# Alabuta/RaytracingInOneWeekend

Hardware: AMD Instinct MI355X
Metric: Mrays/sec + frame wall-clock, huge-scene 1280x720x128spp @1/2/4/8 GPU (higher is better)
Workload: dtype f32; 1 GPU; huge-scene 1280x720x128spp (BASELINE config 3); scene=huge (486 spheres), width=1280, height=720, spp=128, max_depth=64, camera=reference, kernel=exact (bit-exact), cull, parallelism=row-interleaved x1, RCCL gather of f32 tiles, output=f32, hw_queues=8, hw_queues_env=4, deep_split=8, deep_min_items=33554432

## Files before the change

### raytracinginoneweekend_amd/csrc/rt_kernel.hip

```cpp
#include <hip/hip_runtime.h>
#include <float.h>
#include <stdint.h>

#include "rt_device.h"

namespace rt {

#define RT_TMIN 0.008f
#define RT_TMAX FLT_MAX

struct f3 { float x, y, z; };
__device__ __forceinline__ f3 mk(float x, float y, float z) { return {x, y, z}; }
__device__ __forceinline__ f3 operator+(f3 a, f3 b) { return {a.x + b.x, a.y + b.y, a.z + b.z}; }
__device__ __forceinline__ f3 operator-(f3 a, f3 b) { return {a.x - b.x, a.y - b.y, a.z - b.z}; }
__device__ __forceinline__ f3 operator*(f3 a, f3 b) { return {a.x * b.x, a.y * b.y, a.z * b.z}; }
__device__ __forceinline__ f3 operator*(f3 a, float s) { return {a.x * s, a.y * s, a.z * s}; }
__device__ __forceinline__ f3 operator/(f3 a, float s) { return {a.x / s, a.y / s, a.z / s}; }
__device__ __forceinline__ f3 adds(f3 a, float s) { return {a.x + s, a.y + s, a.z + s}; }
__device__ __forceinline__ float dot(f3 a, f3 b) { return a.x * b.x + a.y * b.y + a.z * b.z; }
__device__ __forceinline__ float length(f3 a) { return sqrtf(a.x * a.x + a.y * a.y + a.z * a.z); }
__device__ __forceinline__ f3 normalize(f3 a)
{
    float l = length(a);
    return fabsf(l) > FLT_MIN ? a / l : a;
// ... 1269 lines not shown
                        }
                    }
                }
            }
            stamp(3);
        }
        if constexpr (COUNT) {
            uint32_t r = trap_rem;
            for (int off = 32; off >= 1; off >>= 1) r += (uint32_t)__shfl_xor((int)r, off);
            wt.add_seg(r);
        }
        if (done) {
            RT_EV(EV_STORE);
            finish(col);
        }
    }

    if (COUNT && p.segments) {
        if (lane == 0) {
            atomicAdd(p.segments + 0, (unsigned long long)wt.seg);
            atomicAdd(p.segments + 1, (unsigned long long)wt.sph);
            atomicAdd(p.segments + 2, (unsigned long long)wt.box);
        }
    }
    if (STATS && p.dbg) {
        const uint32_t c[8] = {dbg_iters, dbg_refills, dbg.wave_blocks, dbg.lane_blocks, dbg.wave_roots,
                               dbg.lane_roots, lane == 0 ? (uint32_t)wt.seg : 0u, dbg.wave_member_blocks};
#pragma unroll
        for (int i = 0; i < 8; ++i) {
            unsigned long long v = c[i];
            for (int off = 32; off >= 1; off >>= 1) v += __shfl_xor(v, off);
            if (lane == 0) atomicAdd(p.dbg + i, v);
        }
#pragma unroll
        for (int i = 0; i < (int)EV_COUNT; ++i) {
            unsigned long long v = dbg.ev[i];
            for (int off = 32; off >= 1; off >>= 1) v += __shfl_xor(v, off);
            if (lane == 0) atomicAdd(p.dbg + kDbgEvBase + i, v);
        }
        if (lane == 0) {
            for (int i = 0; i < 5; ++i) atomicAdd(p.dbg + 8 + i, (unsigned long long)cyc[i]);
            atomicMax(p.dbg + 14, ~t_wave0);
            atomicAdd(p.dbg + 13, (unsigned long long)dbg_dealt);
        }
        const uint32_t w = blockIdx.x * (blockDim.x >> 6) + (threadIdx.x >> 6);
        if (lane == 0 && w < kDbgWaves) {
            const unsigned long long cy = cyc[0] + cyc[1] + cyc[2] + cyc[3] + cyc[4];
            p.dbg[16 + 4 * w] = DEEP ? ((unsigned long long)dbg_walks_nohint << 32 | dbg_walks)
                                     : (t_dry ? t_dry : __builtin_amdgcn_s_memrealtime());
            p.dbg[17 + 4 * w] = __builtin_amdgcn_s_memrealtime();
            p.dbg[18 + 4 * w] = (min(cy, 0xffffffffull) << 32) | (min(dbg_refills, 65535u) << 16) | min(dbg_iters, 65535u);
            p.dbg[19 + 4 * w] = ((unsigned long long)(__smid() & 0xffffu) << 48) |
                                ((unsigned long long)min(DEEP ? dbg_walks : dbg_iters_dry, 65535u) << 32) | (uint32_t)t_wave0;
        }
    }
}

template <int V, int CULL, bool STATS, bool COUNT, bool PAIRS = false>
__global__ __launch_bounds__(256, (kMinWaves<V, CULL, STATS>)) void render_kernel(const KParams p)
{
    render_body<V, CULL, STATS, COUNT, false, 4, PAIRS>(p);
}
template <int V, bool STATS, bool COUNT, int WPB>
__global__ __launch_bounds__(64 * WPB, (WPB == 8 && !STATS ? RT_DEEP_WIDE_WAVES : kMinWaves<V, 7, STATS>)) void render_deep_kernel(const KParams p)
{
    render_body<V, 7, STATS, COUNT, true, WPB, false>(p);
}

__device__ __forceinline__ float xs_gen(uint32_t &st)
{
    st ^= st << 13;
    st ^= st >> 17;
    st ^= st << 5;
    return (float)st * (1.f / 4294967296.f);
}
__device__ __forceinline__ f3 xs_unit_sphere(uint32_t &st)
{
    f3 v;
    do {
        const float x = xs_gen(st) * 2.f - 1.f;
        const float y = xs_gen(st) * 2.f - 1.f;
        const float z = xs_gen(st) * 2.f - 1.f;
        v = mk(x, y, z);
    } while (v.x * v.x + v.y * v.y + v.z * v.z > 0x1.000002p+0f && st != 0u);
    return v;
}

__global__ __launch_bounds__(256) void compat_kernel(const KCompat p)
{
    const uint32_t lane = threadIdx.x & 63u;
    const float4 *shade = p.shade;
    const uint8_t *kinds = reinterpret_cast<const uint8_t *>(shade + 2 * p.n_spheres);
    const f3 org = mk(p.org[0], p.org[1], p.org[2]), llc = mk(p.llc[0], p.llc[1], p.llc[2]);
    const f3 hor = mk(p.hor[0], p.hor[1], p.hor[2]), ver = mk(p.ver[0], p.ver[1], p.ver[2]);
    const float fW = (float)p.W, fH = (float)p.H;

    uint32_t cnext = 0, cend = 0;
    bool exhausted = false, alive = false, fresh = false;
    uint32_t i = 0, x = 0, y = 0, s = 0, depth = 0, rng = 0;
    f3 o = mk(0.f, 0.f, 0.f), d = o, att = o, col = o;
    uint32_t segs = 0, tests = 0;
    for (;;) {
        uint64_t need = ballot(!alive);
        while (need && !exhausted) {
            if (cnext >= cend) {
                uint32_t c = 0;
                if (lane == 0) c = atomicAdd(p.ctr, 1u);
                c = __builtin_amdgcn_readfirstlane(c);
                if (c >= p.n_chunks) { exhausted = true; break; }
                cnext = c * 64u;
                cend = min(cnext + 64u, p.n_pixels);
            }
            const uint32_t avail = cend - cnext;
            const uint32_t rank = __builtin_amdgcn_mbcnt_hi((uint32_t)(need >> 32),
                                                            __builtin_amdgcn_mbcnt_lo((uint32_t)need, 0u));
            if (!alive && rank < avail) {
                i = cnext + rank;
                const uint32_t rr = i / p.W;
                x = i - rr * p.W;
                y = p.row_offset + rr * p.row_stride;
                rng = x + y * p.W + p.seed;
                s = 0;
                col = mk(0.f, 0.f, 0.f);
                alive = fresh = true;
            }
            cnext += min((uint32_t)__popcll(need), avail);
            need = ballot(!alive);
        }
        if (ballot(alive) == 0) break;
        if (!alive) continue;
        if (fresh) {
            const float u = ((float)x + xs_gen(rng)) / fW;
            const float v = ((float)y + xs_gen(rng)) / fH;
            o = org;
            d = (llc + hor * u) + ver * (1.f - v);
            att = mk(1.f, 1.f, 1.f);
            depth = 0;
            fresh = false;
        }
        bool done = false;
        f3 c = mk(0.f, 0.f, 0.f);
        if (depth >= p.max_depth) {
            done = true;
        } else {
            ++segs;
            const float a = d.x * d.x + d.y * d.y + d.z * d.z;
            float tmax = RT_TMAX;
            uint32_t ib = 0xffffffffu;
            for (uint32_t k = 0; k < p.n_spheres; ++k) {
                const float4 sf = shade[2 * k];
                const float ocx = o.x - sf.x, ocy = o.y - sf.y, ocz = o.z - sf.z;
                const float b = ocx * d.x + ocy * d.y + ocz * d.z;
                const float cc = ocx * ocx + ocy * ocy + ocz * ocz - sf.w * sf.w;
                const float disc = b * b - a * cc;
                if (disc > 0.f) {
                    const float q = sqrtf(disc);
                    float t = (-b - q) / a;
                    if (!(t < tmax && t > RT_TMIN)) t = (-b + q) / a;
                    if (t < tmax && t > RT_TMIN) { tmax = t; ib = k; }
                }
            }
            tests += p.n_spheres;
            ++depth;
            if (ib == 0xffffffffu) {
                const float tt = normalize(d).y * .5f + .5f;
                c = (mk(1.f, 1.f, 1.f) * (1.f - tt) + mk(.5f, .7f, 1.f) * tt) * att;
                done = true;
            } else {
                const float4 sf = shade[2 * ib], md = shade[2 * ib + 1];
                const uint32_t kind = kinds[ib];
                const f3 hp = o + d * tmax;
                const f3 hn = (hp - mk(sf.x, sf.y, sf.z)) / sf.w;
                bool valid = true;
                f3 nd;
                if (kind == 0u) {
                    nd = hn + normalize(xs_unit_sphere(rng));
                } else if (kind == 1u) {
                    const f3 refl = reflect(normalize(d), hn);
                    nd = refl + normalize(xs_unit_sphere(rng)) * md.w;
                    valid = dot(nd, hn) > 0.f;
                } else {
                    const f3 ud = normalize(d);
                    f3 outward = mk(-hn.x, -hn.y, -hn.z);
                    float ri = md.w;
                    float cosv = dot(ud, hn);
                    if (cosv <= 0.f) {
                        outward = outward * -1.f;
                        ri = 1.f / ri;
                        cosv *= -1.f;
                    }
                    const f3 refr = refract(ud, outward, ri);
                    float prob = 1.f;
                    if (refr.x * refr.x + refr.y * refr.y + refr.z * refr.z > 0.f) prob = schlick(ri, cosv);
                    nd = xs_gen(rng) < prob ? reflect(ud, hn) : refr;
                }
                if (!valid) {
                    done = true;
                } else {
                    o = hp;
                    d = nd;
                    att = att * mk(md.x, md.y, md.z);
                    if (depth >= p.max_depth) done = true;
                }
            }
        }
        if (done) {
            col = col + c;
            if (++s == p.spp) {
                col = col / (float)p.spp;
                const uint32_t row = p.full_frame ? y : i / p.W;
                float *dst = p.out + ((size_t)row * p.W + x) * 3u;
                dst[0] = col.x;
                dst[1] = col.y;
                dst[2] = col.z;
                alive = false;
            } else {
                fresh = true;
            }
        }
    }
    if (p.segments) {
        const unsigned long long cv[2] = {segs, tests};
        for (int k = 0; k < 2; ++k) {
            unsigned long long v = cv[k];
            for (int off = 32; off >= 1; off >>= 1) v += __shfl_xor(v, off);
            if (lane == 0) atomicAdd(p.segments + k, v);
        }
    }
}

__global__ __launch_bounds__(256) void accumulate_kernel(const KAccum k)
{
    const uint32_t i = blockIdx.x * blockDim.x + threadIdx.x;
    if (i == 0 && k.seg_to)
        for (int c = 0; c < 3; ++c) {
            k.seg_to[c] += k.seg_from[c];
            k.seg_from[c] = 0ull;
        }
    if (k.queue_reset)
        for (uint32_t w = i; w < k.queue_words; w += gridDim.x * blockDim.x) {
            if (k.deep_over && (w & (kQueueStride - 1u)) == kDeepCount && k.queue_reset[w] > k.deep_rcap)
                *k.deep_over = k.deep_key;
            k.queue_reset[w] = 0u;
        }
    if (i >= k.n_pixels) return;
    const bool sky = i >= k.sky_pos0;
    if (sky) {
        if (!k.last || k.part == 1) return;
    } else if (k.part) {
        const bool flagged = k.deep_px[i];
        if (k.part == 1 && flagged) return;
        if (k.part == 2 && !flagged) return;
        if (k.part != 1 && flagged) k.deep_px[i] = 0;
    }
    const uint32_t ni = k.block_perm ? (k.block_perm[i >> 6] << 6) | (i & 63u) : i;
    f3 acc;
    if (sky) acc = mk(k.slots[3 * i], k.slots[3 * i + 1], k.slots[3 * i + 2]);
    else if (k.first) acc = mk(0.f, 0.f, 0.f);
    else acc = mk(k.acc[3 * ni], k.acc[3 * ni + 1], k.acc[3 * ni + 2]);
    auto ld = [&](uint32_t s) {
        const float *v = k.slots + ((size_t)s * k.n_pixels + i) * 3u;
        return mk(v[0], v[1], v[2]);
    };
    if (sky) {
    } else if (k.paired) {
        for (uint32_t b = 0; b < k.n_blocks; ++b) acc = acc + (ld(2u * b) + ld(2u * b + 1u));
        for (uint32_t t = 4u * k.n_blocks; t < k.n_samples; ++t) acc = acc + ld(t - 2u * k.n_blocks);
    } else {
        uint32_t s = 0;
        for (; s < 4u * k.n_blocks; s += 4u) acc = acc + ((ld(s) + ld(s + 1u)) + (ld(s + 2u) + ld(s + 3u)));
        for (; s < k.n_samples; ++s) acc = acc + ld(s);
    }
    if (!k.last) {
        k.acc[3 * ni] = acc.x; k.acc[3 * ni + 1] = acc.y; k.acc[3 * ni + 2] = acc.z;
        return;
    }
    const f3 col = acc / (float)k.spp;
    uint32_t x, rr;
    {
        const uint32_t tiled_px = k.tiled_rows * k.W;
        if (ni < tiled_px) {
            uint32_t t = ni >> 6, w = ni & 63u;
            uint32_t ty = t / k.tiles_x, tx = t - ty * k.tiles_x;
            x = (tx << k.tile_lw) + (w & ((1u << k.tile_lw) - 1u));
            rr = (ty << (6u - k.tile_lw)) + (w >> k.tile_lw);
        } else {
            uint32_t jj = ni - tiled_px;
            rr = jj / k.W;
            x = jj - rr * k.W;
            rr += k.tiled_rows;
        }
    }
    const uint32_t row = k.full_frame ? k.row_offset + rr * k.row_stride : rr;
    const size_t o = ((size_t)row * k.W + x) * 3u;
    k.out[o] = col.x; k.out[o + 1] = col.y; k.out[o + 2] = col.z;
    if (k.out_u8) {
        const double g = (double)(1.f / 2.2f);
        k.out_u8[o] = (uint8_t)(255.f * (float)pow((double)col.x, g));
        k.out_u8[o + 1] = (uint8_t)(255.f * (float)pow((double)col.y, g));
        k.out_u8[o + 2] = (uint8_t)(255.f * (float)pow((double)col.z, g));
    }
}

#ifndef RT_SKY_CAP
#define RT_SKY_CAP 2
#endif
__global__ __launch_bounds__(256) void sky_kernel(const KSky p)
{
    const FrameConsts &fc = p.fc;
    const uint32_t t = blockIdx.x * 256u + threadIdx.x;
    const bool live = t < p.n_pix;
    uint32_t px, rr;
    pixel_of(fc, p.pos0 + (live ? t : 0u), px, rr, p.block_perm);
    const uint32_t py = fc.row_offset + rr * fc.row_stride;
    const uint64_t inc_data = ((uint64_t)fc.inc_data_hi << 32) | fc.inc_data_lo;
    const uint64_t inc_cam = ((uint64_t)fc.inc_cam_hi << 32) | fc.inc_cam_lo;
    const uint64_t key0 = (uint64_t)(py * fc.W + px) * fc.spp;
    const uint32_t spp = fc.spp, full_end = spp & ~3u;
    const float fW = fc.fW, fH = fc.fH, rW = fc.rW, rH = fc.rH;
    const bool dw = fc.div_fast & 1u, dh = fc.div_fast & 2u;
    const f3 org = mk(fc.org[0], fc.org[1], fc.org[2]), llc = mk(fc.llc[0], fc.llc[1], fc.llc[2]);
    const f3 hor = mk(fc.hor[0], fc.hor[1], fc.hor[2]), ver = mk(fc.ver[0], fc.ver[1], fc.ver[2]);
    f3 acc = mk(0.f, 0.f, 0.f), pa = acc, pb = acc;
    uint32_t s = live ? 0u : spp;
    bool started = false;
    uint64_t rc = 0;
    float uu = 0.f, vv = 0.f;
    Dbg dbg{};
    const uint64_t cd1 = inc_data * (kPcgMul + 1u), cd2 = cd1 * kPcgMul + inc_data, cc = inc_cam * (kPcgMul + 1u);
    const uint64_t mm = kPcgMul * kPcgMul;
    uint64_t km = key0 * kPcgMul, kmm = km * kPcgMul;
    const float ux = div_const((float)px, fW, rW, dw), vy = div_const((float)py, fH, rH, dh);
    while (ballot(s < spp)) {
        if (s < spp) {
            if (!started) {
                rc = km + cc;
                const float xu = fminf((float)pcg_out(km + cd1), 0x1.fffffep31f) * 0x1p-32f;
                const float xv = fminf((float)pcg_out(kmm + cd2), 0x1.fffffep31f) * 0x1p-32f;
                uu = ux + div_const(xu, fW, rW, dw);
                vv = vy + div_const(xv, fH, rH, dh);
                km += kPcgMul;
                kmm += mm;
                started = true;
            }
            bool got;
            const f3 r = random_in_unit_sphere_capped<false, RT_SKY_CAP>(rc, inc_cam, got, dbg);
            if (got) {
                const f3 rd = r * fc.lens;
                const f3 off = mk(uu * rd.x, vv * rd.y, 0.f);
                f3 d = ((llc + hor * uu) + ver * (1.f - vv)) - off;
                if (fc.corrected) d = d - org;
                const float a = d.x * d.x + d.y * d.y + d.z * d.z;
                float uy;
                if (!ballot(!(a >= 0x1p-40f && a <= 0x1p40f))) {
                    const float l = sqrt_scaled(a);
                    const float y0 = __builtin_amdgcn_rcpf(l);
                    uy = div_ray(d.y, RayDiv{l, fmaf(fmaf(-l, y0, 1.f), y0, y0), 1u});
                } else {
                    uy = normalize(d).y;
                }
                const float tt = .5f * uy + 1.f;
                const f3 col = mk(1.f, 1.f, 1.f) * (1.f - tt) + mk(.5f, .7f, 1.f) * tt;
                const bool tail = s >= full_end;
                const uint32_t j = s & 3u;
                const f3 sum = pa + col;
                const bool odd = !tail && (j & 1u);
                pa = mk(odd ? sum.x : col.x, odd ? sum.y : col.y, odd ? sum.z : col.z);
                const bool first_pair = !tail && j == 1u;
                pb = mk(first_pair ? pa.x : pb.x, first_pair ? pa.y : pb.y, first_pair ? pa.z : pb.z);
                const bool fold = tail || j == 3u;
                const f3 add = pb + pa;
                const f3 fa = acc + mk(tail ? col.x : add.x, tail ? col.y : add.y, tail ? col.z : add.z);
                acc = mk(fold ? fa.x : acc.x, fold ? fa.y : acc.y, fold ? fa.z : acc.z);
                ++s;
                started = false;
            }
        }
    }
    if (live) {
        float *o = p.sums + 3u * (size_t)t;
        o[0] = acc.x;
        o[1] = acc.y;
        o[2] = acc.z;
    }
    if (p.segments) {
        const uint32_t n = lanes(live);
        if ((threadIdx.x & 63u) == 0u && n) atomicAdd(p.segments, (unsigned long long)n * spp);
    }
}

__global__ __launch_bounds__(256) void epilogue_rgb8_kernel(const float *in, uint8_t *out, uint64_t n)
{
    const uint64_t i = (uint64_t)blockIdx.x * blockDim.x + threadIdx.x;
    if (i >= n) return;
    const double g = (double)(1.f / 2.2f);
    out[i] = (uint8_t)(255.f * (float)pow((double)in[i], g));
}

__global__ __launch_bounds__(256) void wave_gen_kernel(const KWave w)
{
    const KParams &p = w.p;
    const FrameConsts &fc = p.fc;
    const uint32_t gid = blockIdx.x * 256u + threadIdx.x;
    if (gid >= w.n_chunk) return;
    const uint32_t I = w.item_begin + gid;
    const uint32_t ls = udiv(I, fc.div_n_pixels);
    const uint32_t pix = I - ls * fc.n_pixels;
    uint32_t px, rr;
    pixel_of(fc, pix, px, rr, nullptr);
    const uint32_t py = fc.row_offset + rr * fc.row_stride;
    const uint32_t sm = fc.sample_begin + ls;
    const uint64_t inc_data = ((uint64_t)fc.inc_data_hi << 32) | fc.inc_data_lo;
    const uint64_t inc_cam = ((uint64_t)fc.inc_cam_hi << 32) | fc.inc_cam_lo;
    const uint64_t km = ((uint64_t)(py * fc.W + px) * fc.spp + sm) * kPcgMul;
    uint64_t rng = km + inc_data * (kPcgMul + 1u);
    uint64_t rc = km + inc_cam * (kPcgMul + 1u);
    const bool fw = fc.div_fast & 1u, fh = fc.div_fast & 2u;
    const float u = div_const((float)px, fc.fW, fc.rW, fw);
    const float v = div_const((float)py, fc.fH, fc.rH, fh);
    const float uu = u + div_const(canonical(rng, inc_data), fc.fW, fc.rW, fw);
    const float vv = v + div_const(canonical(rng, inc_data), fc.fH, fc.rH, fh);
    const f3 r = random_in_unit_sphere(rc, inc_cam);
    const f3 rd = r * fc.lens;
    const f3 off = mk(uu * rd.x, vv * rd.y, 0.f);
    const f3 org = mk(fc.org[0], fc.org[1], fc.org[2]);
    const f3 o = org + off;
    f3 d = ((mk(fc.llc[0], fc.llc[1], fc.llc[2]) + mk(fc.hor[0], fc.hor[1], fc.hor[2]) * uu) +
            mk(fc.ver[0], fc.ver[1], fc.ver[2]) * (1.f - vv)) - off;
    if (fc.corrected) d = d - org;
    const RayQueue &q = w.out;
    q.f[0 * w.cap + gid] = o.x; q.f[1 * w.cap + gid] = o.y; q.f[2 * w.cap + gid] = o.z;
    q.f[3 * w.cap + gid] = d.x; q.f[4 * w.cap + gid] = d.y; q.f[5 * w.cap + gid] = d.z;
    q.f[6 * w.cap + gid] = 1.f; q.f[7 * w.cap + gid] = 1.f; q.f[8 * w.cap + gid] = 1.f;
    q.rng[gid] = rng;
    q.item[gid] = I;
    q.depth[gid] = 0u;
    if (gid == 0) *q.count = w.n_chunk;
}

template <int CULL, bool COUNT>
__global__ __launch_bounds__(256, 6) void wave_bounce_kernel(const KWave w)
{
    const KParams &p = w.p;
    extern __shared__ float4 lds_blob[];
    for (uint32_t i = threadIdx.x; i < p.lds_units; i += blockDim.x) lds_blob[i] = p.blob[i];
    __syncthreads();
    const float4 *blob = lds_blob;
    const float4 *geo = blob;
    const uint32_t *sidx = reinterpret_cast<const uint32_t *>(blob + p.n_geo);
    const float4 *clus = blob + p.clus_offset;
    __shared__ TransposeLds s_tw[4];
    TransposeLds *tw = &s_tw[threadIdx.x >> 6];
    const uint64_t inc_data = ((uint64_t)p.fc.inc_data_hi << 32) | p.fc.inc_data_lo;
    const RayQueue &qi = w.in, &qo = w.out;
    const uint32_t n = *qi.count;
    const uint32_t cap = w.cap;
    WaveTally<COUNT> wt;
    Dbg dbg{};
    for (uint32_t base = blockIdx.x * 256u; base < n; base += gridDim.x * 256u) {
        const uint32_t j = base + threadIdx.x;
        const bool live = j < n;
        const uint32_t jj = live ? j : 0u;
        f3 o = mk(qi.f[0 * cap + jj], qi.f[1 * cap + jj], qi.f[2 * cap + jj]);
        f3 d = mk(qi.f[3 * cap + jj], qi.f[4 * cap + jj], qi.f[5 * cap + jj]);
        f3 att = mk(qi.f[6 * cap + jj], qi.f[7 * cap + jj], qi.f[8 * cap + jj]);
        uint64_t rng = qi.rng[jj];
        const uint32_t I = qi.item[jj];
        uint32_t depth = qi.depth[jj];
        const bool seg = live && depth < p.max_depth;
        const float a = d.x * d.x + d.y * d.y + d.z * d.z;
        const uint64_t segm = ballot(seg);
        const RayDiv rd = ray_div(a, segm, p.fast_roots);
        Hit h = closest_hit<false, CULL, false, COUNT>(p, geo, sidx, clus, o, d, rd, dbg, wt, seg, segm, CULL ? tw : nullptr,
                                                        no_hit());
        if (!seg) h = Hit{kNoHit};
        {
            const uint32_t ns = lanes(seg);
            wt.add_seg(ns);
            wt.add_sph((uint64_t)ns * p.n_always);
        }
        bool done = false, cont = false;
        f3 col = mk(0.f, 0.f, 0.f);
        if (live) {
            if (!seg) {
                done = true;
            } else {
                const float t = h.t();
                const uint32_t ib = h.id();
                ++depth;
                if (ib == 0xffffffffu) {
                    float uy;
                    if (rd.fd != 0u) {
                        const float l = sqrt_scaled(a);
                        const float y0 = __builtin_amdgcn_rcpf(l);
                        uy = div_ray(d.y, RayDiv{l, fmaf(fmaf(-l, y0, 1.f), y0, y0), 1u});
                    } else {
                        uy = normalize(d).y;
                    }
                    const float tt = .5f * uy + 1.f;
                    const f3 bg = mk(1.f, 1.f, 1.f) * (1.f - tt) + mk(.5f, .7f, 1.f) * tt;
                    col = bg * att;
                    done = true;
                } else if (depth >= p.max_depth) {
                    done = true;
                } else {
                    float4 sf, md;
                    uint32_t kind;
                    if (p.shade_lds) {
                        const float4 *shade = blob + p.shade_offset;
                        sf = shade[2 * ib];
                        md = shade[2 * ib + 1];
                        kind = reinterpret_cast<const uint8_t *>(shade + 2 * p.n_spheres)[ib];
                        asm volatile("");
                    } else {
                        const float4 *shade = p.blob + p.shade_offset;
                        sf = gld4(shade, 2 * ib);
                        md = gld4(shade, 2 * ib + 1);
                        kind = ((const __attribute__((address_space(1))) uint8_t *)(shade + 2 * p.n_spheres))[ib];
                    }
                    const f3 hp = o + d * t;
                    const f3 dv = hp - mk(sf.x, sf.y, sf.z);
                    f3 hn;
                    if (p.fast_roots && all_lanes_min_abs_ok(dv)) hn = div3_short(dv, sf.w);
                    else hn = dv / sf.w;
                    att = att * mk(md.x, md.y, md.z);
                    o = hp;
                    cont = true;
                    if (kind == 0u) {
                        const f3 pn = hp + hn;
                        const f3 r = random_in_unit_sphere(rng, inc_data);
                        d = (pn + r) - hp;
                    } else {
                        f3 ud;
                        if (rd.fd != 0u && all_lanes_min_abs_ok(d)) ud = div3_short(d, sqrt_scaled(a));
                        else ud = normalize(d);
                        const f3 rf = reflect(ud, hn);
                        if (kind == 1u) {
                            const f3 r = random_in_unit_sphere(rng, inc_data);
                            const f3 nd = rf + r * md.w;
                            if (dot(nd, hn) > 0.f) {
                                d = nd;
                            } else {
                                cont = false;
                                done = true;
                            }
                        } else {
                            const uint32_t di = p.shade_offset + 2 * p.n_spheres + (p.n_spheres + 15u) / 16u + ib;
                            float4 dcs;
                            if (p.shade_lds) {
                                dcs = blob[di];
                                asm volatile("");
                            } else {
                                dcs = gld4(p.blob, di);
                            }
                            f3 outward = mk(-hn.x, -hn.y, -hn.z);
                            float ri = md.w, xs = dcs.y;
                            float cosv = dot(ud, hn);
                            if (cosv <= 0.f) {
                                outward = outward * -1.f;
                                ri = dcs.x;
                                xs = dcs.z;
                                cosv *= -1.f;
                            }
                            const f3 refr = refract(ud, outward, ri);
                            float prob = 1.f;
                            if (refr.x * refr.x + refr.y * refr.y + refr.z * refr.z > 0.f) prob = schlick_x(xs, cosv);
                            d = canonical(rng, inc_data) < prob ? rf : refr;
                        }
                    }
                }
            }
        }
        if (done) {
            float *dst = p.slots + (size_t)I * 3u;
            dst[0] = col.x;
            dst[1] = col.y;
            dst[2] = col.z;
        }
        const uint64_t cm = ballot(cont);
        if (cm) {
            uint32_t b0 = 0;
            if ((threadIdx.x & 63u) == (uint32_t)__builtin_ctzll(cm)) b0 = atomicAdd(qo.count, (uint32_t)__popcll(cm));
            b0 = __builtin_amdgcn_readlane(b0, __builtin_ctzll(cm));
            if (cont) {
                const uint32_t k = b0 + __builtin_amdgcn_mbcnt_hi((uint32_t)(cm >> 32), __builtin_amdgcn_mbcnt_lo((uint32_t)cm, 0u));
                qo.f[0 * cap + k] = o.x; qo.f[1 * cap + k] = o.y; qo.f[2 * cap + k] = o.z;
                qo.f[3 * cap + k] = d.x; qo.f[4 * cap + k] = d.y; qo.f[5 * cap + k] = d.z;
                qo.f[6 * cap + k] = att.x; qo.f[7 * cap + k] = att.y; qo.f[8 * cap + k] = att.z;
                qo.rng[k] = rng;
                qo.item[k] = I;
                qo.depth[k] = depth;
            }
        }
    }
    if (COUNT && p.segments && (threadIdx.x & 63u) == 0u) {
        atomicAdd(p.segments + 0, (unsigned long long)wt.seg);
        atomicAdd(p.segments + 1, (unsigned long long)wt.sph);
        atomicAdd(p.segments + 2, (unsigned long long)wt.box);
    }
}

template <int V, bool STATS, bool COUNT> static const void *ptr_cull(int cull, bool pairs)
{
    if (cull == 7) return pairs ? reinterpret_cast<const void *>(&render_kernel<V, 7, STATS, COUNT, true>)
                                : reinterpret_cast<const void *>(&render_kernel<V, 7, STATS, COUNT>);
    return pairs ? nullptr : reinterpret_cast<const void *>(&render_kernel<V, 0, STATS, COUNT>);
}

template <bool COUNT> static const void *render_ptr_c(int variant, int cull, bool pairs)
{
    switch (variant) {
    case V_EXACT_LDS: return ptr_cull<V_EXACT_LDS, false, COUNT>(cull, pairs);
    case V_FAST_LDS: return ptr_cull<V_FAST_LDS, false, COUNT>(cull, pairs);
    case V_EXACT_SCALAR:
        return cull || pairs ? nullptr : reinterpret_cast<const void *>(&render_kernel<V_EXACT_SCALAR, 0, false, COUNT>);
    case V_STATS_LDS: return ptr_cull<V_EXACT_LDS, true, true>(cull, pairs);
    default: return nullptr;
    }
}
static const void *render_ptr(int variant, int cull, bool count, bool pairs = false)
{
    return count ? render_ptr_c<true>(variant, cull, pairs) : render_ptr_c<false>(variant, cull, pairs);
}

template <bool COUNT, int WPB> static const void *render_deep_ptr_w(int variant)
{
    switch (variant) {
    case V_EXACT_LDS: return reinterpret_cast<const void *>(&render_deep_kernel<V_EXACT_LDS, false, COUNT, WPB>);
    case V_FAST_LDS: return reinterpret_cast<const void *>(&render_deep_kernel<V_FAST_LDS, false, COUNT, WPB>);
    case V_STATS_LDS: return reinterpret_cast<const void *>(&render_deep_kernel<V_EXACT_LDS, true, true, WPB>);
    default: return nullptr;
    }
}
static const void *render_deep_ptr(int variant, bool count, int wpb)
{
    if (wpb == 8) return count ? render_deep_ptr_w<true, 8>(variant) : render_deep_ptr_w<false, 8>(variant);
    if (wpb == 4) return count ? render_deep_ptr_w<true, 4>(variant) : render_deep_ptr_w<false, 4>(variant);
    return nullptr;
}

hipError_t launch_render(int variant, int cull, const KParams &p, uint32_t grid, hipStream_t stream, int wpb)
{
    const bool count = p.segments != nullptr;
    const void *fn = p.deep_mode ? (cull == 7 ? render_deep_ptr(variant, count, wpb) : nullptr)
                                 : (wpb == 4 ? render_ptr(variant, cull, count, p.n_pair_items != 0) : nullptr);
    if (!fn) return hipErrorInvalidValue;
    const size_t lds = (size_t)p.lds_units * 16u;
    void *args[] = {const_cast<KParams *>(&p)};
    return hipLaunchKernel(fn, dim3(grid), dim3(64u * (uint32_t)wpb), args, lds, stream);
}

hipError_t deep_occupancy(int variant, int wpb, size_t lds, int *blocks_per_cu, size_t *static_lds)
{
    const void *fn = render_deep_ptr(variant, false, wpb);
    if (!fn) return hipErrorInvalidValue;
    hipFuncAttributes a{};
    hipError_t e = hipFuncGetAttributes(&a, fn);
    if (e != hipSuccess) return e;
    *static_lds = a.sharedSizeBytes;
    return hipOccupancyMaxActiveBlocksPerMultiprocessor(blocks_per_cu, fn, 64 * wpb, lds);
}

hipError_t occupancy_render(int variant, int cull, int *blocks_per_cu, size_t lds, bool pairs)
{
    const void *fn = render_ptr(variant, cull, false, pairs);
    if (!fn) return hipErrorInvalidValue;
    return hipOccupancyMaxActiveBlocksPerMultiprocessor(blocks_per_cu, fn, 256, lds);
}

hipError_t static_lds_render(int variant, int cull, size_t *bytes, bool pairs)
{
    const void *fn = render_ptr(variant, cull, false, pairs);
    if (!fn) return hipErrorInvalidValue;
    hipFuncAttributes a{};
    const hipError_t e = hipFuncGetAttributes(&a, fn);
    if (e == hipSuccess) *bytes = a.sharedSizeBytes;
    return e;
}

// ... 62 lines not shown
```

Before: 60510 Mrays/s.

## Decouple sky-kernel lens rejection sampling from shading via shared-memory ring

The sky kernel's per-lane rejection-sampling loop for lens offsets is split from the shading step. Lanes draw accepted lens samples ahead into a per-thread shared-memory ring buffer. Shading then runs in warp-uniform lockstep over sample index, with uniform accumulation branches. This aims to reduce divergence caused by lanes needing different numbers of rejection retries, at the cost of shared memory, extra LDS traffic and a more intricate control flow.

```diff
diff --git a/raytracinginoneweekend_amd/csrc/rt_kernel.hip b/raytracinginoneweekend_amd/csrc/rt_kernel.hip
--- a/raytracinginoneweekend_amd/csrc/rt_kernel.hip
+++ b/raytracinginoneweekend_amd/csrc/rt_kernel.hip
@@ -1595,11 +1595,16 @@
     }
 }
 
-#ifndef RT_SKY_CAP
-#define RT_SKY_CAP 2
+#ifndef RT_SKY_RING
+#define RT_SKY_RING 8
 #endif
+#ifndef RT_SKY_VCONST
+#define RT_SKY_VCONST 0
+#endif
+static_assert(RT_SKY_RING >= 2 && (RT_SKY_RING & (RT_SKY_RING - 1)) == 0, "ring depth: a power of two");
 __global__ __launch_bounds__(256) void sky_kernel(const KSky p)
 {
+    __shared__ float2 ring[RT_SKY_RING][256];
     const FrameConsts &fc = p.fc;
     const uint32_t t = blockIdx.x * 256u + threadIdx.x;
     const bool live = t < p.n_pix;
@@ -1610,64 +1615,82 @@
     const uint64_t inc_cam = ((uint64_t)fc.inc_cam_hi << 32) | fc.inc_cam_lo;
     const uint64_t key0 = (uint64_t)(py * fc.W + px) * fc.spp;
     const uint32_t spp = fc.spp, full_end = spp & ~3u;
-    const float fW = fc.fW, fH = fc.fH, rW = fc.rW, rH = fc.rH;
+    float fW = fc.fW, fH = fc.fH, rW = fc.rW, rH = fc.rH, lens = fc.lens;
     const bool dw = fc.div_fast & 1u, dh = fc.div_fast & 2u;
-    const f3 org = mk(fc.org[0], fc.org[1], fc.org[2]), llc = mk(fc.llc[0], fc.llc[1], fc.llc[2]);
-    const f3 hor = mk(fc.hor[0], fc.hor[1], fc.hor[2]), ver = mk(fc.ver[0], fc.ver[1], fc.ver[2]);
+    f3 org = mk(fc.org[0], fc.org[1], fc.org[2]), llc = mk(fc.llc[0], fc.llc[1], fc.llc[2]);
+    f3 hor = mk(fc.hor[0], fc.hor[1], fc.hor[2]), ver = mk(fc.ver[0], fc.ver[1], fc.ver[2]);
+    if (RT_SKY_VCONST >= 1) asm volatile("" : "+v"(fW), "+v"(fH), "+v"(rW), "+v"(rH), "+v"(lens));
+    if (RT_SKY_VCONST >= 2) {
+        asm volatile("" : "+v"(org.x), "+v"(org.y), "+v"(org.z), "+v"(llc.x), "+v"(llc.y), "+v"(llc.z));
+        asm volatile("" : "+v"(hor.x), "+v"(hor.y), "+v"(hor.z), "+v"(ver.x), "+v"(ver.y), "+v"(ver.z));
+    }
     f3 acc = mk(0.f, 0.f, 0.f), pa = acc, pb = acc;
-    uint32_t s = live ? 0u : spp;
-    bool started = false;
-    uint64_t rc = 0;
-    float uu = 0.f, vv = 0.f;
-    Dbg dbg{};
     const uint64_t cd1 = inc_data * (kPcgMul + 1u), cd2 = cd1 * kPcgMul + inc_data, cc = inc_cam * (kPcgMul + 1u);
     const uint64_t mm = kPcgMul * kPcgMul;
     uint64_t km = key0 * kPcgMul, kmm = km * kPcgMul;
     const float ux = div_const((float)px, fW, rW, dw), vy = div_const((float)py, fH, rH, dh);
-    while (ballot(s < spp)) {
-        if (s < spp) {
-            if (!started) {
-                rc = km + cc;
-                const float xu = fminf((float)pcg_out(km + cd1), 0x1.fffffep31f) * 0x1p-32f;
-                const float xv = fminf((float)pcg_out(kmm + cd2), 0x1.fffffep31f) * 0x1p-32f;
-                uu = ux + div_const(xu, fW, rW, dw);
-                vv = vy + div_const(xv, fH, rH, dh);
-                km += kPcgMul;
-                kmm += mm;
-                started = true;
-            }
-            bool got;
-            const f3 r = random_in_unit_sphere_capped<false, RT_SKY_CAP>(rc, inc_cam, got, dbg);
-            if (got) {
-                const f3 rd = r * fc.lens;
-                const f3 off = mk(uu * rd.x, vv * rd.y, 0.f);
-                f3 d = ((llc + hor * uu) + ver * (1.f - vv)) - off;
-                if (fc.corrected) d = d - org;
-                const float a = d.x * d.x + d.y * d.y + d.z * d.z;
-                float uy;
-                if (!ballot(!(a >= 0x1p-40f && a <= 0x1p40f))) {
-                    const float l = sqrt_scaled(a);
-                    const float y0 = __builtin_amdgcn_rcpf(l);
-                    uy = div_ray(d.y, RayDiv{l, fmaf(fmaf(-l, y0, 1.f), y0, y0), 1u});
-                } else {
-                    uy = normalize(d).y;
+    uint32_t sd = live ? 0u : spp;
+    uint64_t rc = km + cc, kc = km + kPcgMul;
+    uint32_t m_lo = (uint32_t)kPcgMul, m_hi = (uint32_t)(kPcgMul >> 32);
+    float k31 = 0x1p-31f;
+    asm volatile("" : "+v"(m_lo), "+v"(m_hi), "+v"(k31));
+    const uint64_t mul = ((uint64_t)m_hi << 32) | m_lo;
+    auto draw = [&]() {
+        const uint64_t old = rc;
+        rc = old * mul + inc_cam;
+        return fmaf(fminf((float)pcg_out(old), 0x1.fffffep31f), k31, -1.f);
+    };
+    const uint32_t n_s = ballot(live) ? spp : 0u;
+    const uint32_t tid = threadIdx.x;
+    for (uint32_t sc = 0; sc < n_s;) {
+        if (ballot(sd == sc)) {
+            const uint32_t room_end = min(spp, sc + (uint32_t)RT_SKY_RING);
+            if (sd < room_end) {
+                const float x = draw();
+                const float y = draw();
+                const float z = draw();
+                if (!(x * x + y * y + z * z > 0x1.000002p+0f)) {
+                    ring[sd & (RT_SKY_RING - 1u)][tid] = make_float2(x, y);
+                    ++sd;
+                    rc = kc + cc;
+                    kc += kPcgMul;
                 }
-                const float tt = .5f * uy + 1.f;
-                const f3 col = mk(1.f, 1.f, 1.f) * (1.f - tt) + mk(.5f, .7f, 1.f) * tt;
-                const bool tail = s >= full_end;
-                const uint32_t j = s & 3u;
-                const f3 sum = pa + col;
-                const bool odd = !tail && (j & 1u);
-                pa = mk(odd ? sum.x : col.x, odd ? sum.y : col.y, odd ? sum.z : col.z);
-                const bool first_pair = !tail && j == 1u;
-                pb = mk(first_pair ? pa.x : pb.x, first_pair ? pa.y : pb.y, first_pair ? pa.z : pb.z);
-                const bool fold = tail || j == 3u;
-                const f3 add = pb + pa;
-                const f3 fa = acc + mk(tail ? col.x : add.x, tail ? col.y : add.y, tail ? col.z : add.z);
-                acc = mk(fold ? fa.x : acc.x, fold ? fa.y : acc.y, fold ? fa.z : acc.z);
-                ++s;
-                started = false;
-            }
+            }
+        }
+        if (!ballot(sd == sc)) {
+            const float2 r = ring[sc & (RT_SKY_RING - 1u)][tid];
+            const float xu = fminf((float)pcg_out(km + cd1), 0x1.fffffep31f) * 0x1p-32f;
+            const float xv = fminf((float)pcg_out(kmm + cd2), 0x1.fffffep31f) * 0x1p-32f;
+            const float uu = ux + div_const(xu, fW, rW, dw);
+            const float vv = vy + div_const(xv, fH, rH, dh);
+            km += kPcgMul;
+            kmm += mm;
+            const f3 rd = mk(r.x * lens, r.y * lens, 0.f);
+            const f3 off = mk(uu * rd.x, vv * rd.y, 0.f);
+            f3 d = ((llc + hor * uu) + ver * (1.f - vv)) - off;
+            if (fc.corrected) d = d - org;
+            const float a = d.x * d.x + d.y * d.y + d.z * d.z;
+            float uy;
+            if (!ballot(!(a >= 0x1p-40f && a <= 0x1p40f))) {
+                const float l = sqrt_scaled(a);
+                const float y0 = __builtin_amdgcn_rcpf(l);
+                uy = div_ray(d.y, RayDiv{l, fmaf(fmaf(-l, y0, 1.f), y0, y0), 1u});
+            } else {
+                uy = normalize(d).y;
+            }
+            const float tt = .5f * uy + 1.f;
+            const f3 col = mk(1.f, 1.f, 1.f) * (1.f - tt) + mk(.5f, .7f, 1.f) * tt;
+            const uint32_t j = sc & 3u;
+            if (sc >= full_end) {
+                acc = acc + col;
+            } else if (j == 1u) {
+                pb = pa + col;
+            } else if (j == 3u) {
+                acc = acc + (pb + (pa + col));
+            } else {
+                pa = col;
+            }
+            ++sc;
         }
     }
     if (live) {
```

New measurement: 63740 Mrays/s (median of 6 runs). +5.3%, better.
